# ankitkumar93/compute-war

Hardware: AMD Instinct MI355X
Metric: GB/s ingested (Skein-512 + LZ4, 64 KiB blocks) (higher is better)
Workload: dtype u64; 1 GPU; skein512+lz4, 1048576 x 65536 B uniform-random blocks/GPU in HBM; blocks_per_gpu=1048576, block_bytes=65536, parallelism=block-sharded x1, gather-only RCCL

## Files before the change

### compute_war_amd/csrc/cdc_kernels.hip

```cpp

#include <hip/hip_runtime.h>
#include <stdint.h>

#include "cdc_resolve.h"
#include "cw_device.h"
#include "stream_scratch.h"

namespace cw {

namespace {

constexpr unsigned kScanThreads = 512;

template <bool HI, bool EDGE>
__device__ __forceinline__ void scan_slice(const uint64_t *__restrict__ tab, unsigned copy, const uint8_t *__restrict__ base,
                                           uint64_t last_granule, uint64_t q0, uint64_t off, uint64_t nv, uint64_t ms, uint64_t ml,
                                           uint64_t &ws, uint64_t &wl)
{
    const uint32_t msh = (uint32_t)(ms >> 32), msl = (uint32_t)ms, mlh = (uint32_t)(ml >> 32), mll = (uint32_t)ml;
    auto granule = [&](int i) __attribute__((always_inline)) {
        const int64_t gi = (int64_t)(q0 >> 4) - 4 + i;
        const uint64_t g = gi < 0 ? 0 : ((uint64_t)gi > last_granule ? last_granule : (uint64_t)gi);
        return *reinterpret_cast<const uint4 *>(base + g * 16);
    };
    uint64_t h = 0, s = 0, l = 0;
    uint4 cur = granule(0);
#pragma unroll 1
    for (int i = 0; i < 8; i++) {
        const uint4 nxt = granule(i + 1 < 8 ? i + 1 : 7);
        const uint32_t d[4] = {cur.x, cur.y, cur.z, cur.w};
#pragma unroll
        for (int j = 0; j < 16; j++) {
            const uint32_t b = (d[j >> 2] >> (8 * (j & 3))) & 0xFF;
            uint64_t g = tab[(b << 5) | copy];
            const int pos = 16 * i + j - 64;
// ... 3 lines not shown
                const uint32_t hh = (uint32_t)(h >> 32), hl = (uint32_t)h;
                bool cs = (hh & msh) == 0, cl = (hh & mlh) == 0;
                if (!HI) { cs = cs && (hl & msl) == 0; cl = cl && (hl & mll) == 0; }
                if (EDGE) {
                    const uint64_t q = q0 + pos;
                    const bool in = q >= off && q < nv;
                    cs = cs && in; cl = cl && in;
                }
                s |= (uint64_t)cs << pos;
                l |= (uint64_t)cl << pos;
            }
        }
        cur = nxt;
    }
    ws = s;
    wl = l;
}

template <bool HI>
__global__ void __launch_bounds__(kScanThreads)
cdc_scan_kernel(const uint8_t *__restrict__ base, uint64_t off, uint64_t n, const uint64_t *__restrict__ gear, uint64_t ms, uint64_t ml,
                uint64_t *__restrict__ l0s, uint64_t *__restrict__ l0l, uint64_t *__restrict__ l1, uint64_t nwords, uint64_t nspans)
{
    __shared__ uint64_t tab[256 * 32];
    for (unsigned i = threadIdx.x; i < 256 * 32; i += blockDim.x) tab[i] = gear[i >> 5];
    __syncthreads();
    const unsigned lane = threadIdx.x & 63, copy = threadIdx.x & 31;
    const uint64_t nv = n + off, last_granule = (nv - 1) >> 4;
    const uint64_t waves = (uint64_t)gridDim.x * (kScanThreads / 64);
    for (uint64_t span = (uint64_t)blockIdx.x * (kScanThreads / 64) + (threadIdx.x >> 6); span < nspans; span += waves) {
        const uint64_t word = span * 64 + lane, q0 = word * 64;
        const bool edge = span == 0 || (span + 1) * 4096 > nv;
        uint64_t ws, wl;
        if (edge) scan_slice<HI, true>(tab, copy, base, last_granule, q0, off, nv, ms, ml, ws, wl);
        else scan_slice<HI, false>(tab, copy, base, last_granule, q0, off, nv, ms, ml, ws, wl);
        const bool have = word < nwords;
        if (have) { l0s[word] = ws; l0l[word] = wl; }
        const uint64_t b0 = __ballot(have && ws != 0), b1 = __ballot(have && wl != 0);
        const uint64_t b2 = __ballot(have && ws != ~0ull), b3 = __ballot(have && wl != ~0ull);
        if (lane == 0) {
            l1[span * 4 + 0] = b0; l1[span * 4 + 1] = b1; l1[span * 4 + 2] = b2; l1[span * 4 + 3] = b3;
        }
    }
}

__global__ void __launch_bounds__(256)
cdc_summary_kernel(const uint64_t *__restrict__ in, uint64_t nin, uint64_t *__restrict__ out, uint64_t nout)
// ... 110 lines not shown
    const size_t nstreams = st ? st->nstreams : 0;
    hipError_t e = space.reserve(st ? cdc_streams_workspace_bytes(nbytes, nstreams, p.min_size, seg) : cdc_workspace_bytes(nbytes, p.min_size, seg), kFloor);
    if (e != hipSuccess) return e;
    uint8_t *w = space.as<uint8_t>();
    auto take = [&](size_t bytes) { uint8_t *r = w; w += up256(bytes); return r; };
    uint64_t *gear = reinterpret_cast<uint64_t *>(take(2048));
    uint64_t *l0 = reinterpret_cast<uint64_t *>(take(2 * nwords * 8));
    uint64_t *lv = reinterpret_cast<uint64_t *>(take(4 * 8 * (n1 + n2 + n3)));
    const uint64_t cuts = nseg * cap + nstreams;
    uint64_t *segs = reinterpret_cast<uint64_t *>(take(2 * cuts * 8 + 2 * nseg * 8 + (nseg + 63) / 64 * 8 + 3 * nseg * 4));
    uint64_t *notmerged = segs + 2 * cuts + 2 * nseg;
    uint32_t *counts = reinterpret_cast<uint32_t *>(take(nseg * 4));
    uint64_t *segoff = reinterpret_cast<uint64_t *>(take((nseg + 1) * 8));
    uint32_t *eidx = st ? reinterpret_cast<uint32_t *>(take((nseg + 1) * 4)) : nullptr;

    e = hipMemcpyAsync(gear, p.gear, 2048, hipMemcpyHostToDevice, stream);
    if (e == hipSuccess) e = hipMemsetAsync(notmerged, 0, (nseg + 63) / 64 * 8, stream);
    if (e != hipSuccess) return e;
    if (st) {
        if ((e = cdc_streams_verdict_launch(*st, nbytes, seg, nseg, eidx, offsets, nchunks, stream)) != hipSuccess) return e;
    }
    const bool hi = (uint32_t)p.mask_s == 0 && (uint32_t)p.mask_l == 0;
    const unsigned scan_grid = (unsigned)(n1 < 4096 ? (n1 + 7) / 8 : 512);
    if (hi) hipLaunchKernelGGL((cdc_scan_kernel<true>), dim3(scan_grid), dim3(kScanThreads), 0, stream, base, off, (uint64_t)nbytes, gear,
                               p.mask_s, p.mask_l, l0, l0 + nwords, lv, nwords, n1);
    else hipLaunchKernelGGL((cdc_scan_kernel<false>), dim3(scan_grid), dim3(kScanThreads), 0, stream, base, off, (uint64_t)nbytes, gear,
                            p.mask_s, p.mask_l, l0, l0 + nwords, lv, nwords, n1);
    uint64_t *l1 = lv, *l2 = lv + 4 * n1, *l3 = lv + 4 * (n1 + n2);
    hipLaunchKernelGGL(cdc_summary_kernel, dim3((unsigned)umin((n2 + 3) / 4, 1024)), dim3(256), 0, stream, l1, n1, l2, n2);
    hipLaunchKernelGGL(cdc_summary_kernel, dim3((unsigned)umin((n3 + 3) / 4, 1024)), dim3(256), 0, stream, l2, n2, l3, n3);

    CdcS c;
    c.l0 = l0; c.lv = lv;
    c.nwords = nwords; c.n1 = n1; c.n2 = n2; c.off = off; c.n = nbytes; c.seg = seg; c.nseg = nseg;
    c.m = p.min_size; c.a = p.normal_size; c.M = p.max_size; c.cap = (uint32_t)cap; c.final_ = final_;
    c.segs = segs;
    const unsigned sg = (unsigned)((nseg + 63) / 64), cg = (unsigned)((nseg + 255) / 256);
    if (st) {
        c.ends = st->ends; c.eidx = eidx; c.verdict = st->result; c.nstreams = nstreams;
        if ((e = cdc_streams_resolve_launch(c, counts, stream)) != hipSuccess) return e;
    } else {
        const Cdc &c1 = c;
        hipLaunchKernelGGL(cdc_spec_kernel<Cdc>, dim3(sg), dim3(64), 0, stream, c1, nseg);
        hipLaunchKernelGGL(cdc_merge_kernel<Cdc>, dim3(sg), dim3(64), 0, stream, c1, nseg);
        hipLaunchKernelGGL(cdc_fixup_kernel<Cdc>, dim3(1), dim3(64), 0, stream, c1, nseg);
        hipLaunchKernelGGL(cdc_count_kernel<Cdc>, dim3(cg), dim3(256), 0, stream, c1, nseg, counts);
    }
    e = hipGetLastError();
    if (e != hipSuccess) return e;
// ... 53 lines not shown
```

### compute_war_amd/csrc/cw_api.hip

```cpp

#include <atomic>
#include <cstdarg>
#include <cstdio>
#include <cstdlib>
#include <cstring>
#include <memory>
#include <mutex>
#include <string>
#include <vector>

#include "cw_host.h"
#include "launch_plan.h"

using namespace cw::host;

namespace {
thread_local char t_err[512] = "";

struct ProfSpan { int kind; hipEvent_t a, b; };
thread_local bool t_prof_on = false;
thread_local std::vector<ProfSpan> t_prof;
}

int cw::host::fail(int code, const char *fmt, ...)
// ... 624 lines not shown
{
    int rc = ensure_init();
    if (rc != CW_OK) return rc;
    HIP_TRY(hipMemcpy(dst, d_src, bytes, hipMemcpyDeviceToHost));
    return CW_OK;
}
int cw_dev_synchronize(void)
{
    int rc = ensure_init();
    if (rc != CW_OK) return rc;
    HIP_TRY(hipDeviceSynchronize());
    return CW_OK;
}

#ifdef CW_CLOCK_STAMP
int cw_debug_clock_read(int which, unsigned long long *out)
{
    int rc = ensure_init();
    if (rc != CW_OK) return rc;
    HIP_TRY(hipDeviceSynchronize());
    HIP_TRY(which == 0 ? cw::skein_clock_read(out) : cw::lz4_clock_read(out));
    return CW_OK;
}
#endif

void cw_profile_enable(int on) { t_prof_on = on != 0; }

int cw_profile_read(double ms_sum[3], unsigned count[3], int reset)
{
    for (int k = 0; k < PROF_KINDS; k++) { ms_sum[k] = 0; count[k] = 0; }
    for (ProfSpan &p : t_prof) {
        float ms = 0;
        HIP_TRY(hipEventSynchronize(p.b));
        HIP_TRY(hipEventElapsedTime(&ms, p.a, p.b));
        ms_sum[p.kind] += ms;
        count[p.kind]++;
    }
    if (reset) {
        for (ProfSpan &p : t_prof) { (void)hipEventDestroy(p.a); (void)hipEventDestroy(p.b); }
        t_prof.clear();
    }
    return CW_OK;
}

int cw_profile_kernels(int kind, char *buf, size_t cap)
{
// ... 492 lines not shown
```

### compute_war_amd/csrc/cw_device.h

```cpp
#pragma once

#include <hip/hip_runtime.h>
#include <stddef.h>
#include <stdint.h>

#include "knobs.h"

#ifndef CW_SKEIN_THREADS
#define CW_SKEIN_THREADS 64
#endif

namespace cw {

#ifdef CW_CLOCK_STAMP
constexpr unsigned kClockSlots = 1024;
struct ClockScope {
    unsigned long long m0 = 0, r0 = 0;
    unsigned long long *rec;
    bool on;
    __device__ ClockScope(unsigned long long *buf, unsigned wg) : rec(buf + 4 * (wg % kClockSlots)), on(threadIdx.x == 0)
    {
        if (on) { m0 = __builtin_amdgcn_s_memtime(); r0 = __builtin_amdgcn_s_memrealtime(); }
    }
    __device__ ~ClockScope()
    {
        if (on) {
            const unsigned long long m1 = __builtin_amdgcn_s_memtime(), r1 = __builtin_amdgcn_s_memrealtime();
            rec[0] = m0; rec[1] = r0; rec[2] = m1; rec[3] = r1;
        }
    }
};
#define CW_CLOCK_SCOPE(buf) ClockScope clock_scope_(buf, blockIdx.x)
#define CW_CLOCK_SCOPE_KEYED(buf, key) ClockScope clock_scope_(buf, ((unsigned)(key) % 8u) * 128u + blockIdx.x % 128u)
hipError_t skein_clock_read(unsigned long long *out);
hipError_t lz4_clock_read(unsigned long long *out);
#else
#define CW_CLOCK_SCOPE(buf) do { } while (0)
#define CW_CLOCK_SCOPE_KEYED(buf, key) do { } while (0)
#endif

struct SkeinIV { uint64_t w[8]; };

void note_kernels(int kind, const char *names);
void skein_compute_iv(int state_words, unsigned hash_bits, SkeinIV *iv, uint64_t tree_info = 0);
hipError_t skein_tree_launch(int state_words, const uint8_t *src, size_t block_bytes, size_t src_stride, size_t nblocks,
                             unsigned hash_bits, unsigned leaf, unsigned node, unsigned max_level, uint8_t *digests, hipStream_t stream);

struct HashPlan;
hipError_t skein_launch(const HashPlan &p, const uint8_t *src, size_t block_bytes, size_t src_stride, size_t nblocks, const SkeinIV &iv,
                        uint8_t *digests, unsigned digest_bytes, hipStream_t stream);
hipError_t sha256_launch(const HashPlan &p, const uint8_t *src, size_t block_bytes, size_t src_stride, size_t nblocks, uint8_t *digests,
                         hipStream_t stream);
struct AfterScan { hipError_t (*fn)(void *ctx); void *ctx; };
hipError_t lz4_launch(const uint8_t *src, size_t block_bytes, size_t src_stride, size_t nblocks, uint8_t *dst,
                      size_t dst_stride, uint32_t *sizes, hipStream_t stream, const AfterScan *after_scan = nullptr);
const uint32_t *lz4_queued_blocks_word(hipStream_t stream);
hipError_t lzf_launch(const uint8_t *src, size_t block_bytes, size_t src_stride, size_t nblocks, uint8_t *dst,
                      size_t dst_stride, uint32_t *sizes, hipStream_t stream);
enum class Lz4Vtab : uint8_t;
hipError_t lz4_vtab_launch(Lz4Vtab kernel, uint32_t grid, uint32_t lds, hipStream_t stream, const uint8_t *src, uint32_t n, size_t src_stride, uint8_t *dst,
                           size_t dst_stride, uint32_t *sizes, const uint32_t *queue, uint32_t *counters, uint32_t min_queued, uint32_t max_queued,
// ... 176 lines not shown
```

### compute_war_amd/csrc/launch_plan.h

```cpp
#pragma once

#include <stddef.h>
#include <stdint.h>
#include <stdlib.h>

#include <string>
#include <vector>

#include "knobs.h"

namespace cw {

constexpr uint32_t kTabBytes = (1u << 13) * 2;
constexpr uint32_t kStageMax = 16384;
constexpr uint32_t kFpBytes = (1u << 13) / 2;
constexpr uint32_t kChunk = 4096;
constexpr uint32_t kLzfTabBytes = (1u << 16) * 2;
constexpr uint32_t kInLdsMax = 16384;
constexpr uint32_t kChainMax = 16384;
constexpr uint32_t kShareSpinCap = 1u << 20;

enum class Lz4ScanSpan : uint8_t { unaligned, aligned };
enum class Lz4Parse : uint8_t { global, staged, fp8, fp16, fp32 };
enum class Lz4Lanes : uint8_t { plain, tagged, fp };
enum class Lz4Ring : uint8_t { k1, k2, k4, k8 };
enum class Lz4Blocks : uint8_t { global, staged };
enum class Lz4Vtab : uint8_t { gen2, gen3, lds_table };
enum class LzfLanes : uint8_t { plain, tagged };
enum class LzfChain : uint8_t { small, big, sthread };
enum class LzfParse : uint8_t { global, staged };

template <class E, class Fn>
struct KernelRow { E id; const char *name; Fn *fn; };
template <class E, class Fn, size_t N>
inline const KernelRow<E, Fn> &kernel_row(const KernelRow<E, Fn> (&table)[N], E id)
{
    for (const auto &r : table)
        if (r.id == id) return r;
    abort();
// ... 134 lines not shown
```

### compute_war_amd/csrc/lz4_kernel.hip

```cpp

#include <hip/hip_runtime.h>
#include <stdint.h>
#include <stdio.h>
#include <stdlib.h>
#include <string.h>

#include <optional>
#include <type_traits>

#include "cw_device.h"
#include "lane_codec.h"
#include "launch_plan.h"
#include "lz_device.h"
#include "stream_scratch.h"

#ifndef HEADW_GLOBAL
#define HEADW_GLOBAL 16
#endif
#ifndef HEADW_STAGED
#define HEADW_STAGED 64
#endif

namespace cw {

// ... 43 lines not shown
    const uint32_t n255 = extra / 255;
    for (uint32_t i = lane; i < n255; i += 64) g[i] = 255;
    if (lane == 0) g[n255] = (uint8_t)(extra - n255 * 255);
    return n255 + 1;
}


__device__ __forceinline__ uint32_t ld32g(const uint8_t *p)
{
    uint32_t v;
    __builtin_memcpy(&v, p, 4);
    return v;
}

}

struct ScanState {
    bool hit = false, maybe = false;
    uint32_t mcand = 0, mv = 0;
};

__device__ __forceinline__ uint32_t scan_issue(uint32_t *tab, uint32_t tag, uint32_t pos, uint32_t v, bool active)
{
    const uint32_t h = v * 2654435761u, fp = (h >> 7) & 0xFFFu;
    return atomicMax(&tab[active ? h >> 19 : 0u], active ? tag | (pos << 12) | fp : 0u);
}
__device__ __forceinline__ void scan_judge(uint32_t old, uint32_t epoch, uint32_t v0, uint32_t pos, uint32_t v, bool active, ScanState &st)
{
    const uint32_t fp = ((v * 2654435761u) >> 7) & 0xFFFu, cand = (old >> 12) & 0xFFFFu;
    const bool same = (old >> 28) == epoch;
    const bool fpm = active && same && (old & 0xFFFu) == fp;
    st.hit |= active && (same ? cand >= pos : v == v0);
    st.hit |= fpm && st.maybe;
    st.mcand = fpm ? cand : st.mcand;
    st.mv = fpm ? v : st.mv;
    st.maybe |= fpm;
}

__device__ __forceinline__ bool scan_settle(const uint8_t *g, ScanState &st)
{
    if (__ballot(st.maybe)) {
        if (st.maybe) st.hit |= ld32g(g + st.mcand) == st.mv;
        st.maybe = false;
    }
    return __ballot(st.hit) != 0;
}

__device__ __forceinline__ void scan_begin_block(uint32_t *tab, uint32_t &epoch, uint32_t lane)
{
    if (++epoch == 16) {
        for (uint32_t i = lane; i < (1u << 13) / 4; i += 64) reinterpret_cast<uint4 *>(tab)[i] = make_uint4(0, 0, 0, 0);
        epoch = 1;
    }
}

struct BlockFeed {
// ... 6 lines not shown
        __syncthreads();
        if (lane == 0) *mailbox = atomicAdd(&counters[2], run);
        __syncthreads();
        f.next = __builtin_amdgcn_readfirstlane(*mailbox);
        f.end = f.next + run;
    }
    blk = f.next++;
    return blk < nblocks;
}

__device__ __forceinline__ void scan_mark(uint32_t *sizes, size_t blk, uint32_t *queue, uint32_t *counters, uint32_t lane)
{
    if (lane == 0) {
        sizes[blk] = kNeedsParse;
        queue[atomicAdd(&counters[1], 1u)] = (uint32_t)blk;
    }
}

__global__ void __launch_bounds__(64)
lz4_scan_kernel(const uint8_t *__restrict__ src, uint32_t n, size_t src_stride, size_t nblocks,
                        uint8_t *__restrict__ dst, size_t dst_stride, uint32_t *__restrict__ sizes, uint32_t nprobes,
                        uint32_t *__restrict__ queue, uint32_t *__restrict__ counters)
{
    __shared__ __attribute__((aligned(16))) uint32_t tab[1u << 13];
    __shared__ __attribute__((aligned(16))) uint32_t mailbox_word[4];
    volatile uint32_t *mailbox = mailbox_word;
    const uint32_t lane = threadIdx.x;
    __builtin_amdgcn_s_setprio(3);
    uint32_t epoch = 15;

    BlockFeed feed;
    const uint32_t run = n >= 65536 ? 1u : 65536u / n;
    for (size_t blk; scan_next_block(feed, blk, counters, mailbox, run, nblocks, lane);) {
        scan_begin_block(tab, epoch, lane);
        const uint8_t *g = src + blk * src_stride;
        uint8_t *out = dst + blk * dst_stride;
        const uint32_t tag = epoch << 28;
        ScanState st;
        bool marked = false;

        if (nprobes) {
            const uint32_t v0 = ld32g(g);
            {
                const uint32_t h0 = v0 * 2654435761u;
                if (lane == 0) atomicMax(&tab[h0 >> 19], tag | ((h0 >> 7) & 0xFFFu));
            }
            for (uint32_t k0 = 0; k0 < nprobes && !marked; k0 += 64 * kScanGroup) {
                uint32_t pos[kScanGroup], v[kScanGroup];
                bool act[kScanGroup];
#pragma unroll
                for (int j = 0; j < kScanGroup; j++) {
                    const uint32_t k = k0 + 64 * j + lane;
                    pos[j] = 1 + probe_delta(k);
                    act[j] = k < nprobes;
                    v[j] = ld32g(g + (act[j] ? pos[j] : 0u));
                }
                uint32_t old[kScanGroup];
#pragma unroll
                for (int j = 0; j < kScanGroup; j++) old[j] = scan_issue(tab, tag, pos[j], v[j], act[j]);
#pragma unroll
                for (int j = 0; j < kScanGroup; j++) scan_judge(old[j], epoch, v0, pos[j], v[j], act[j], st);
                marked = scan_settle(g, st);
            }
        }
        if (marked) {
            scan_mark(sizes, blk, queue, counters, lane);
            continue;
        }
        uint32_t op = 1;
        if (n >= 15) {
            if (lane == 0) out[0] = 15u << 4;
            op += put_len(out + 1, n - 15, lane);
        } else if (lane == 0) {
            out[0] = (uint8_t)(n << 4);
        }
        copy_g2g(out + op, g, n, lane);
        if (lane == 0) sizes[blk] = op + n;
    }
}

constexpr uint32_t kPieces = kChunk / 1024, kRing = 2 * kChunk, kStreamGroup = 2;

struct Chunk { uint4 p[kPieces]; };

__device__ __forceinline__ void chunk_load(Chunk &r, const uint8_t *g, uint32_t c, uint32_t nchunks, uint32_t n, uint32_t lane)
{
#pragma unroll
    for (uint32_t j = 0; j < kPieces; j++) {
        const uint32_t off = c * kChunk + j * 1024 + lane * 16;
        if (c < nchunks && off < n) r.p[j] = *reinterpret_cast<const uint4 *>(g + off);
    }
}
__device__ __forceinline__ void chunk_stage(const Chunk &r, uint32_t *ring32, uint32_t c, uint32_t n, uint32_t lane)
{
#pragma unroll
    for (uint32_t j = 0; j < kPieces; j++) {
        const uint32_t off = c * kChunk + j * 1024 + lane * 16;
        if (off < n) *reinterpret_cast<uint4 *>(reinterpret_cast<uint8_t *>(ring32) + (off & (kRing - 1))) = r.p[j];
    }
}
__device__ __forceinline__ void chunk_store(const Chunk &r, uint8_t *lit, uint32_t c, uint32_t n, uint32_t lane)
{
#pragma unroll
    for (uint32_t j = 0; j < kPieces; j++) {
// ... 40 lines not shown
        for (uint32_t j = 0; j < kStreamGroup; j++) {
            const uint32_t k = w.knext + 64 * j + lane;
            pos[j] = 1 + probe_delta(k);
            act[j] = k < nprobes && pos[j] < end;
            const unsigned long long m = __ballot(act[j]);
            nact += (uint32_t)__builtin_popcountll(m);
            ngroups += m != 0;
        }
        if (nact == 0) return;
        if (ngroups == 1) probe_groups<1>(w, pos, act, tab, ring32, tag, epoch);
        else if (ngroups == 2) probe_groups<2>(w, pos, act, tab, ring32, tag, epoch);
        else probe_groups<kStreamGroup>(w, pos, act, tab, ring32, tag, epoch);
        w.marked = scan_settle(g, w.st);
        w.knext += nact;
        if (w.marked || nact < 64 * kStreamGroup) return;
    }
}

__global__ void __launch_bounds__(64)
lz4_scan_stream_kernel(const uint8_t *__restrict__ src, uint32_t n, size_t src_stride, size_t nblocks,
                       uint8_t *__restrict__ dst, size_t dst_stride, uint32_t *__restrict__ sizes, uint32_t nprobes,
                       uint32_t *__restrict__ queue, uint32_t *__restrict__ counters, size_t first_block, uint32_t feed_word)
{
    __shared__ __attribute__((aligned(16))) uint32_t tab[1u << 13];
    __shared__ __attribute__((aligned(16))) uint32_t ring32[kRing / 4];
    volatile uint32_t *mailbox = ring32;
    const uint32_t lane = threadIdx.x;
    __builtin_amdgcn_s_setprio(3);
    uint32_t epoch = 15;
    const uint32_t nchunks = (n + kChunk - 1) / kChunk;
    const uint32_t hdr = 1 + (n >= 15 ? (n - 15) / 255 + 1 : 0);

    BlockFeed feed;
    const uint32_t run = n >= 65536 ? 1u : 65536u / n;
    for (size_t rel; scan_next_block(feed, rel, counters + feed_word - 2, mailbox, run, nblocks - first_block, lane);) {
        const size_t blk = first_block + rel;
        scan_begin_block(tab, epoch, lane);
        const uint8_t *g = src + blk * src_stride;
        uint8_t *out = dst + blk * dst_stride, *lit = out + hdr;
        const uint32_t tag = epoch << 28;
        Walk w;
        Chunk r0, r1, r2;

#define CW_STAGE(PREV, CUR, C)                                                                         \
        do {                                                                                           \
            const uint32_t c_ = (C);                                                                   \
            if (c_) chunk_store(PREV, lit, c_ - 1, n, lane);                                           \
            chunk_load(PREV, g, c_ + 2, nchunks, n, lane);                                             \
            chunk_stage(CUR, ring32, c_, n, lane);                                                     \
            if (c_ == 0) {                                                                             \
                w.v0 = ring32[0];                                                                      \
                if (nprobes && lane == 0) {                                                            \
                    const uint32_t h0 = w.v0 * 2654435761u;                                            \
                    atomicMax(&tab[h0 >> 19], tag | ((h0 >> 7) & 0xFFFu));             \
                }                                                                                      \
            } else {                                                                                   \
                probe_upto(w, c_ * kChunk, tab, ring32, tag, epoch, nprobes, g, lane);                 \
            }                                                                                          \
// ... 114 lines not shown
    w.marked = probe_batches<1, true>(pos, q ? 0u : 62u, left < 64 ? left : 64u, tab, ring32, tag, w.v0, g, lane);
    w.qnext = q + 1;
}

__device__ __forceinline__ void probe_range(SpanWalk &w, uint32_t qe, uint32_t *tab, const uint32_t *ring32, uint32_t tag, const uint8_t *g,
                                            uint32_t lane)
{
    uint32_t q = w.qnext;
    w.qnext = qe;
    uint32_t p = __umul24(q, lane) + group_base(q);
    for (; q + 2 <= qe; q += 2) {
        const uint32_t pos[2] = {p, p + lane + (64 * q + 1)};
        if (probe_batches<2, false>(pos, 0, 64, tab, ring32, tag, w.v0, g, lane)) { w.marked = true; return; }
        p = pos[1] + lane + (64 * q + 65);
    }
    if (q < qe) {
        const uint32_t pos[1] = {p};
        w.marked = probe_batches<1, false>(pos, 0, 64, tab, ring32, tag, w.v0, g, lane);
    }
}

#ifdef CW_CLOCK_STAMP
__device__ unsigned long long g_clock_scan[4 * kClockSlots];
hipError_t lz4_clock_read(unsigned long long *out) { return hipMemcpyFromSymbol(out, HIP_SYMBOL(g_clock_scan), sizeof g_clock_scan); }
#endif

template <bool ALIGNED>
__global__ void __launch_bounds__(64)
lz4_scan_span_kernel(const uint8_t *__restrict__ src, uint32_t n, size_t src_stride, uint32_t nspans, uint8_t *__restrict__ dst,
                     size_t dst_stride, uint32_t *__restrict__ sizes, uint32_t nprobes, uint32_t *__restrict__ queue,
                     uint32_t *__restrict__ counters, uint32_t lg)
{
    CW_CLOCK_SCOPE(g_clock_scan);
    __shared__ __attribute__((aligned(16))) uint32_t tab[1u << 13];
    __shared__ __attribute__((aligned(16))) uint32_t ring32[kRing / 4];
    volatile uint32_t *mailbox = ring32;
    const uint32_t lane = threadIdx.x;
    __builtin_amdgcn_s_setprio(3);
    uint32_t epoch = 15;
    const uint32_t cmask = (1u << lg) - 1, run = 16u >> lg;
    const uint32_t hdr = 1 + (n - 15) / 255 + 1;
    const uint32_t lane16 = lane * 16;
    const uint32_t qlast = (nprobes + 61) >> 6;
    const uint32_t gend = group_end((lane + 1) * kChunk < n ? (lane + 1) * kChunk : n, qlast);
    const uint32_t hdrw = (0xFFu << 16) | (((n - 15) % 255) << 24);

    for (;;) {
        __syncthreads();
        if (lane == 0) *mailbox = atomicAdd(&counters[2], 1u);
        __syncthreads();
        const uint32_t span = __builtin_amdgcn_readfirstlane(*mailbox);
        if (span >= nspans) break;
        __syncthreads();
        const size_t first = (size_t)span * run;
        const uint8_t *gs = src + first * src_stride;
        uint8_t *os = dst + first * dst_stride + (ALIGNED ? hdr - 2 : hdr);

        SpanWalk w;
// ... 851 lines not shown
        blk = queue[qi];
        g = src + (size_t)blk * src_stride;
        out = dst + (size_t)blk * dst_stride;
        return Take::kTaken;
    }
};

template <int MODE>
__global__ void __launch_bounds__(64)
lz4_lanes_kernel(const uint8_t *__restrict__ src, uint32_t n, size_t src_stride, uint8_t *__restrict__ dst, size_t dst_stride,
                 uint32_t *__restrict__ sizes, const uint32_t *__restrict__ queue, uint32_t *__restrict__ counters,
                 uint16_t *__restrict__ tables, uint32_t min_blocks, uint32_t reserve)
{
    const uint32_t qcount = counters[1];
    if (qcount < min_blocks) return;
    if ((size_t)blockIdx.x * 64 >= qcount) return;
    LaneQueue s{src, src_stride, dst, dst_stride, sizes, queue, counters, qcount, reserve, n, n - kMFLimit, n - kLastLiterals,
                src, dst, 0};
    LaneTab<MODE> t{reinterpret_cast<typename LaneTab<MODE>::Entry *>(tables) + ((size_t)blockIdx.x * 64 + threadIdx.x) * (1u << 13)};
    lz4_lane_run(s, t);
}

constexpr uint32_t kRingBytes = 256, kRingPiece = 64;
enum : uint32_t { LB_NEXT = 0, LB_PROBE = 1, LB_EXTEND = 2, LB_TAIL = 3, LB_EXIT = 4 };

template <int K>
__device__ __forceinline__ void
lz4_lanes_ring_body(uint32_t *__restrict__ ring, const uint32_t qcount, const uint8_t *__restrict__ src, uint32_t n, size_t src_stride, uint8_t *__restrict__ dst,
                    size_t dst_stride, uint32_t *__restrict__ sizes, const uint32_t *__restrict__ queue, uint32_t *__restrict__ counters,
                    uint16_t *__restrict__ tables, uint32_t reserve)
{
    const uint32_t lane = threadIdx.x;
    uint32_t *tab = reinterpret_cast<uint32_t *>(tables) + ((size_t)blockIdx.x * 64 + lane) * (1u << 13);
    const uint32_t mflimit = n - kMFLimit, matchlimit = n - kLastLiterals;

    auto ring_dw = [&](uint32_t x) -> uint32_t { return ring[((x >> 2) & (kRingBytes / 4 - 1)) * 64 + lane]; };
    auto ring32 = [&](uint32_t x) -> uint32_t { return __builtin_amdgcn_alignbyte(ring_dw(x + 4), ring_dw(x), x & 3u); };
    auto ring16 = [&](uint32_t x) -> uint4 {
        const uint32_t d0 = ring_dw(x), d1 = ring_dw(x + 4), d2 = ring_dw(x + 8), d3 = ring_dw(x + 12), d4 = ring_dw(x + 16), r = x & 3u;
        return make_uint4(__builtin_amdgcn_alignbyte(d1, d0, r), __builtin_amdgcn_alignbyte(d2, d1, r), __builtin_amdgcn_alignbyte(d3, d2, r),
                          __builtin_amdgcn_alignbyte(d4, d3, r));
    };

    uint32_t state = LB_NEXT;
    const uint8_t *g = src;
    uint8_t *out = dst;
// ... 228 lines not shown
            const uint32_t run = n - anchor;
            if (run >= 15) { out[op++] = 15u << 4; lane_put_len(out, op, run - 15); }
            else out[op++] = (uint8_t)(run << 4);
            uint32_t k = 0;
            for (; k + 16 <= run; k += 16) {
                uint4 q;
                __builtin_memcpy(&q, g + anchor + k, 16);
                __builtin_memcpy(out + op + k, &q, 16);
            }
            for (; k < run; k++) out[op + k] = g[anchor + k];
            op += run;
            sizes[blk] = op;
            state = LB_NEXT;
        }
    }
}

template <int K>
__global__ void __launch_bounds__(64)
lz4_lanes_ring_kernel(const uint8_t *__restrict__ src, uint32_t n, size_t src_stride, uint8_t *__restrict__ dst, size_t dst_stride,
                      uint32_t *__restrict__ sizes, const uint32_t *__restrict__ queue, uint32_t *__restrict__ counters,
                      uint16_t *__restrict__ tables, uint32_t min_blocks, uint32_t reserve, uint32_t max_blocks)
{
    __shared__ uint32_t ring[(kRingBytes / 4) * 64];
    const uint32_t qcount = counters[1];
    if (qcount < min_blocks || qcount >= max_blocks) return;
    if ((size_t)blockIdx.x * 64 >= qcount) return;
    lz4_lanes_ring_body<K>(ring, qcount, src, n, src_stride, dst, dst_stride, sizes, queue, counters, tables, reserve);
}

__global__ void __launch_bounds__(64)
lz4_lanes_ring_auto_kernel(const uint8_t *__restrict__ src, uint32_t n, size_t src_stride, uint8_t *__restrict__ dst, size_t dst_stride,
                           uint32_t *__restrict__ sizes, const uint32_t *__restrict__ queue, uint32_t *__restrict__ counters,
                           uint16_t *__restrict__ tables, uint32_t min_blocks, uint32_t reserve_mid, uint32_t wide_from, uint32_t reserve_wide,
                           uint32_t leave_mid)
{
    __shared__ uint32_t ring[(kRingBytes / 4) * 64];
    const uint32_t qcount = counters[1];
    if (qcount < min_blocks) return;
    if ((size_t)blockIdx.x * 64 >= qcount) return;
    if (qcount >= wide_from) {
        lz4_lanes_ring_body<1>(ring, qcount, src, n, src_stride, dst, dst_stride, sizes, queue, counters, tables, reserve_wide);
    } else {
        if ((size_t)blockIdx.x * 64 + leave_mid >= qcount && blockIdx.x > 0) return;
        lz4_lanes_ring_body<2>(ring, qcount, src, n, src_stride, dst, dst_stride, sizes, queue, counters, tables, reserve_mid);
    }
}

namespace {
struct Workspace {
    DeviceBuf queues;
    DeviceBuf lane_tabs;
    SideStream lanes;
    SideStream vtab;
    void release() { (void)queues.release(); (void)lane_tabs.release(); lanes.release(); vtab.release(); }
};
StreamScratch<Workspace> workspaces;
}

const uint32_t *lz4_queued_blocks_word(hipStream_t stream)
// ... 50 lines not shown
    if (!lz4_call_valid(block_bytes, nblocks)) return hipErrorInvalidValue;
    const uint32_t n = (uint32_t)block_bytes;
    const Knobs kn = knobs();
    const CodecCall call = codec_call(src, block_bytes, src_stride, nblocks, dst, dst_stride);
    Lz4Plan p = lz4_plan(call, kn);
    hipError_t e = lz4_set_attributes();
    if (e != hipSuccess) return e;
    auto &wsp = workspaces.at(stream);
    LaunchLock sequence(wsp.launch);
    if ((e = wsp.queues.reserve(p.queue_bytes, p.queue_min_bytes)) != hipSuccess) return e;
    if (p.lanes.on && wsp.lane_tabs.reserve(p.lane_tab_bytes) != hipSuccess) {
        (void)hipGetLastError();
        p = lz4_plan(call, kn, false);
    }
    const size_t cap = (wsp.queues.bytes() / sizeof(uint32_t) - 8) / 2;
    uint32_t *counters = wsp.queues.as<uint32_t>(), *queue = counters + 8, *queue2 = queue + cap;
    uint16_t *const lane_tabs = wsp.lane_tabs.as<uint16_t>();
    std::optional<SideStream::Fork> lanes_fork, vtab_fork;
    auto on = [&](const Stage &s) { return s.stream == Target::lanes_side ? wsp.lanes.stream : s.stream == Target::vtab_side ? wsp.vtab.stream : stream; };
    auto pool = [](SidePool sp) { return sp == SidePool::greatest ? SideStream::greatest : SideStream::normal; };

    if ((e = hipMemsetAsync(counters, 0, 8 * sizeof(uint32_t), stream)) != hipSuccess) return e;
    if (p.scan_span.on)
        hipLaunchKernelGGL(kernel_row(kScanSpanKernels, p.scan_span_kernel).fn, dim3(p.scan_span.grid), dim3(64), 0, stream, src, n, src_stride, p.nspans,
                           dst, dst_stride, sizes, scan_probes(n), queue, counters, p.lg);
    if (p.scan_stream.on)
        hipLaunchKernelGGL(lz4_scan_stream_kernel, dim3(p.scan_stream.grid), dim3(64), 0, stream, src, n, src_stride, nblocks, dst,
                           dst_stride, sizes, scan_probes(n), queue, counters, p.done, 3u);
    if (p.scan_generic.on)
        hipLaunchKernelGGL(lz4_scan_kernel, dim3(p.scan_generic.grid), dim3(64), 0, stream, src, n, src_stride, nblocks, dst,
                           dst_stride, sizes, scan_probes(n), queue, counters);
    if ((e = hipGetLastError()) != hipSuccess) return e;
    if (after_scan && (e = after_scan->fn(after_scan->ctx)) != hipSuccess) return e;
    if (p.stop_after_scan) { note_kernels(0, describe(p).text); return hipSuccess; }
    if (p.lanes.on) {
        if (p.lanes.stream == Target::lanes_side) {
            if ((e = wsp.lanes.open(pool(p.lanes_pool))) != hipSuccess) return e;
            if ((e = lanes_fork.emplace(wsp.lanes, stream).err) != hipSuccess) return e;
        }
        const dim3 lgrid(p.lanes.grid);
        if (p.lanes_form == Lz4Plan::LanesForm::ring_auto)
            hipLaunchKernelGGL(lz4_lanes_ring_auto_kernel, lgrid, dim3(64), 0, on(p.lanes), src, n, src_stride, dst, dst_stride, sizes, queue, counters,
                               lane_tabs, p.lmin, p.reserve, p.wide_from, p.reserve_wide, p.lane_leave);
        else if (p.lanes_form == Lz4Plan::LanesForm::ring)
            hipLaunchKernelGGL(kernel_row(kRingKernels, p.ring_kernel).fn, lgrid, dim3(64), 0, on(p.lanes), src, n, src_stride, dst, dst_stride, sizes, queue,
                               counters, lane_tabs, p.lmin, p.reserve, kNoMax);
        else
            hipLaunchKernelGGL(kernel_row(kLanesKernels, p.lanes_kernel).fn, lgrid, dim3(64), 0, on(p.lanes), src, n, src_stride, dst, dst_stride, sizes, queue,
                               counters, lane_tabs, p.lmin, p.reserve);
        if ((e = hipGetLastError()) != hipSuccess) return e;
    }
    if (p.vtab.on) {
        if (p.vtab.stream == Target::vtab_side) {
            if ((e = wsp.vtab.open(pool(p.vtab_pool))) != hipSuccess) return e;
            if ((e = vtab_fork.emplace(wsp.vtab, stream).err) != hipSuccess) return e;
        }
        if ((e = lz4_vtab_launch(p.vtab_kernel, p.vtab.grid, p.vtab.lds, on(p.vtab), src, n, src_stride, dst, dst_stride, sizes, queue, counters, p.vmin, p.vmax,
                                 p.vres)) != hipSuccess) return e;
    }
    if (p.ltab.on && (e = lz4_vtab_launch(Lz4Vtab::lds_table, p.ltab.grid, p.ltab.lds, stream, src, n, src_stride, dst, dst_stride, sizes, queue, counters, 0u,
                                          kNoMax, 0u)) != hipSuccess) return e;
    if (p.parse.on) {
        hipLaunchKernelGGL(kernel_row(kParseKernels, p.parse_kernel).fn, dim3(p.parse.grid), dim3(64), p.parse.lds, stream, src, n, src_stride, nblocks, dst,
                           dst_stride, sizes, queue, counters, queue2, p.force_redo);
        if ((e = hipGetLastError()) != hipSuccess) return e;
    }
    if (vtab_fork && (e = vtab_fork->join()) != hipSuccess) return e;
    if (lanes_fork && (e = lanes_fork->join()) != hipSuccess) return e;
// ... 9 lines not shown
```

### compute_war_amd/csrc/skein_kernels.hip

```cpp

#include <hip/hip_runtime.h>
#include <stdint.h>
#include <stdlib.h>
#include <string.h>

#include "cw_device.h"
#include "launch_plan.h"
#include "stream_scratch.h"

namespace cw {

#define KS_PARITY 0x5555555555555555ULL

template <int R>
static __device__ __forceinline__ uint64_t rotl(uint64_t x)
{
    const uint32_t lo = (uint32_t)x, hi = (uint32_t)(x >> 32);
    uint32_t nlo, nhi;
    if (R == 32) { nlo = hi; nhi = lo; }
    else if (R < 32) {
        nlo = __builtin_amdgcn_alignbit(lo, hi, 32 - R);
        nhi = __builtin_amdgcn_alignbit(hi, lo, 32 - R);
    } else {
        nlo = __builtin_amdgcn_alignbit(hi, lo, 64 - R);
// ... 269 lines not shown
        fetch_half(S, first + SPL + HS);
        run_half(B, first + HS);
#pragma unroll
        for (unsigned j = 0; j < HS; j++)
#pragma unroll
            for (int k = 0; k < NW; k++) B[j][k] = S[j][k];
    }

    uint8_t *out = digests + gid * digest_bytes;
    if (((digest_bytes | (unsigned)reinterpret_cast<uintptr_t>(out)) & 15) == 0) {
        uint4 *o4 = reinterpret_cast<uint4 *>(out);
#pragma unroll
        for (int k = 0; k < NW / 2; k++)
            if ((unsigned)(16 * k) < digest_bytes)
                o4[k] = make_uint4((uint32_t)X[2 * k], (uint32_t)(X[2 * k] >> 32), (uint32_t)X[2 * k + 1], (uint32_t)(X[2 * k + 1] >> 32));
    } else {
        for (unsigned k = 0; k < digest_bytes; k++) out[k] = (uint8_t)(X[k >> 3] >> (8 * (k & 7)));
    }
}


#ifdef CW_CLOCK_STAMP
__device__ unsigned long long g_clock_skein[4 * kClockSlots];
hipError_t skein_clock_read(unsigned long long *out) { return hipMemcpyFromSymbol(out, HIP_SYMBOL(g_clock_skein), sizeof g_clock_skein); }
#endif

template <int NW, bool ALIGNED16, bool INTERIOR>
__global__ void __launch_bounds__(CW_SKEIN_THREADS)
skein_slice_kernel(const uint8_t *__restrict__ src, size_t block_bytes, size_t src_stride, size_t nblocks, SkeinIV iv,
                   uint8_t *__restrict__ digests, unsigned digest_bytes, uint64_t *__restrict__ state, size_t s_begin, size_t s_end)
{
    CW_CLOCK_SCOPE_KEYED(g_clock_skein, s_begin / (s_end - s_begin ? s_end - s_begin : 1));
    constexpr unsigned BB = NW * 8, SPL = 128 / BB, HS = SPL / 2;
    const size_t gid = (size_t)blockIdx.x * blockDim.x + threadIdx.x;
    if (gid >= nblocks) return;
    const uint8_t *p = src + gid * src_stride;
    const size_t nmsg = block_bytes / BB, total = nmsg + 1;
    uint64_t *st = state + gid * NW;

    uint64_t X[NW];
    if (s_begin == 0) {
#pragma unroll
        for (int i = 0; i < NW; i++) X[i] = iv.w[i];
    } else {
#pragma unroll
        for (int i = 0; i < NW; i++) X[i] = st[i];
    }
    uint64_t t0 = (uint64_t)s_begin * BB, t1 = (s_begin == 0 ? T1_FIRST : 0) | T1_MSG;

    uint64_t A[HS][NW], B[HS][NW], S[HS][NW];
    auto fetch_half = [&](uint64_t (&dst)[HS][NW], size_t first) __attribute__((always_inline)) {
#pragma unroll
        for (unsigned j = 0; j < HS; j++) {
            const size_t s = first + j;
            if constexpr (INTERIOR) {
// ... 353 lines not shown
```

Baseline: 1156 GB/s.

## Move kernel LDS to dynamic shared memory and add clock census instrumentation

Converts the static shared arrays in the CDC scan, LZ4 scan and ring-lane kernels to dynamically sized extern shared memory, with the sizes passed at launch, and registers LDS limits for the CDC scan kernel. Rewrites the scan hash-table issue and judge helpers with branchless masks and bitwise booleans, and uses empty asm barriers to keep the lane id in a vector register. Adds a debug census recorder, enabled only under the clock-stamp build flag, that captures per-workgroup hardware IDs and timestamps. The likely intent is to cut scalar/vector branching overhead and control how shared memory is allocated, at the cost of extra complexity and a risk of mismatched LDS sizes.

```diff
diff --git a/compute_war_amd/csrc/cdc_kernels.hip b/compute_war_amd/csrc/cdc_kernels.hip
--- a/compute_war_amd/csrc/cdc_kernels.hip
+++ b/compute_war_amd/csrc/cdc_kernels.hip
@@ -11,6 +11,7 @@
 namespace {
 
 constexpr unsigned kScanThreads = 512;
+constexpr uint32_t kScanLds = 256 * 32 * 8;
 
 template <bool HI, bool EDGE>
 __device__ __forceinline__ void scan_slice(const uint64_t *__restrict__ tab, unsigned copy, const uint8_t *__restrict__ base,
@@ -60,7 +61,8 @@
 cdc_scan_kernel(const uint8_t *__restrict__ base, uint64_t off, uint64_t n, const uint64_t *__restrict__ gear, uint64_t ms, uint64_t ml,
                 uint64_t *__restrict__ l0s, uint64_t *__restrict__ l0l, uint64_t *__restrict__ l1, uint64_t nwords, uint64_t nspans)
 {
-    __shared__ uint64_t tab[256 * 32];
+    extern __shared__ __attribute__((aligned(16))) uint8_t smem[];
+    uint64_t *const tab = reinterpret_cast<uint64_t *>(smem);
     for (unsigned i = threadIdx.x; i < 256 * 32; i += blockDim.x) tab[i] = gear[i >> 5];
     __syncthreads();
     const unsigned lane = threadIdx.x & 63, copy = threadIdx.x & 31;
@@ -217,9 +219,12 @@
     }
     const bool hi = (uint32_t)p.mask_s == 0 && (uint32_t)p.mask_l == 0;
     const unsigned scan_grid = (unsigned)(n1 < 4096 ? (n1 + 7) / 8 : 512);
-    if (hi) hipLaunchKernelGGL((cdc_scan_kernel<true>), dim3(scan_grid), dim3(kScanThreads), 0, stream, base, off, (uint64_t)nbytes, gear,
+    static std::atomic<bool> lds_set{false};
+    if ((e = set_lds_limits_once(lds_set, {{reinterpret_cast<const void *>(cdc_scan_kernel<true>), kScanLds},
+                                           {reinterpret_cast<const void *>(cdc_scan_kernel<false>), kScanLds}})) != hipSuccess) return e;
+    if (hi) hipLaunchKernelGGL((cdc_scan_kernel<true>), dim3(scan_grid), dim3(kScanThreads), kScanLds, stream, base, off, (uint64_t)nbytes, gear,
                                p.mask_s, p.mask_l, l0, l0 + nwords, lv, nwords, n1);
-    else hipLaunchKernelGGL((cdc_scan_kernel<false>), dim3(scan_grid), dim3(kScanThreads), 0, stream, base, off, (uint64_t)nbytes, gear,
+    else hipLaunchKernelGGL((cdc_scan_kernel<false>), dim3(scan_grid), dim3(kScanThreads), kScanLds, stream, base, off, (uint64_t)nbytes, gear,
                             p.mask_s, p.mask_l, l0, l0 + nwords, lv, nwords, n1);
     uint64_t *l1 = lv, *l2 = lv + 4 * n1, *l3 = lv + 4 * (n1 + n2);
     hipLaunchKernelGGL(cdc_summary_kernel, dim3((unsigned)umin((n2 + 3) / 4, 1024)), dim3(256), 0, stream, l1, n1, l2, n2);
diff --git a/compute_war_amd/csrc/cw_api.hip b/compute_war_amd/csrc/cw_api.hip
--- a/compute_war_amd/csrc/cw_api.hip
+++ b/compute_war_amd/csrc/cw_api.hip
@@ -670,6 +670,14 @@
     HIP_TRY(which == 0 ? cw::skein_clock_read(out) : cw::lz4_clock_read(out));
     return CW_OK;
 }
+int cw_debug_census_read(int which, unsigned long long *out)
+{
+    int rc = ensure_init();
+    if (rc != CW_OK) return rc;
+    HIP_TRY(hipDeviceSynchronize());
+    HIP_TRY(which == 0 ? cw::skein_census_read(out) : cw::lz4_census_read(out));
+    return CW_OK;
+}
 #endif
 
 void cw_profile_enable(int on) { t_prof_on = on != 0; }
diff --git a/compute_war_amd/csrc/cw_device.h b/compute_war_amd/csrc/cw_device.h
--- a/compute_war_amd/csrc/cw_device.h
+++ b/compute_war_amd/csrc/cw_device.h
@@ -14,29 +14,39 @@
 
 #ifdef CW_CLOCK_STAMP
 constexpr unsigned kClockSlots = 1024;
+constexpr unsigned kCensusScan = 1024, kCensusHashLaunch = 16384, kCensusHash = 8 * kCensusHashLaunch;
 struct ClockScope {
-    unsigned long long m0 = 0, r0 = 0;
-    unsigned long long *rec;
+    unsigned long long m0 = 0, r0 = 0, where = 0;
+    unsigned long long *rec, *cen;
     bool on;
-    __device__ ClockScope(unsigned long long *buf, unsigned wg) : rec(buf + 4 * (wg % kClockSlots)), on(threadIdx.x == 0)
+    __device__ ClockScope(unsigned long long *buf, unsigned wg, unsigned long long *census)
+        : rec(buf + 4 * (wg % kClockSlots)), cen(census), on(threadIdx.x == 0)
     {
-        if (on) { m0 = __builtin_amdgcn_s_memtime(); r0 = __builtin_amdgcn_s_memrealtime(); }
+        if (on) {
+            where = (unsigned long long)__builtin_amdgcn_s_getreg((31 << 11) | 4) | (unsigned long long)__builtin_amdgcn_s_getreg((31 << 11) | 20) << 32;
+            m0 = __builtin_amdgcn_s_memtime(); r0 = __builtin_amdgcn_s_memrealtime();
+        }
     }
     __device__ ~ClockScope()
     {
         if (on) {
             const unsigned long long m1 = __builtin_amdgcn_s_memtime(), r1 = __builtin_amdgcn_s_memrealtime();
             rec[0] = m0; rec[1] = r0; rec[2] = m1; rec[3] = r1;
+            cen[0] = r0; cen[1] = r1; cen[2] = m1 - m0; cen[3] = where;
         }
     }
 };
-#define CW_CLOCK_SCOPE(buf) ClockScope clock_scope_(buf, blockIdx.x)
-#define CW_CLOCK_SCOPE_KEYED(buf, key) ClockScope clock_scope_(buf, ((unsigned)(key) % 8u) * 128u + blockIdx.x % 128u)
+#define CW_CLOCK_SCOPE(buf, census) ClockScope clock_scope_(buf, blockIdx.x, (census) + 4 * (blockIdx.x % kCensusScan))
+#define CW_CLOCK_SCOPE_KEYED(buf, census, key)                                                \
+    ClockScope clock_scope_(buf, ((unsigned)(key) % 8u) * 128u + blockIdx.x % 128u,           \
+                            (census) + 4 * (((unsigned)(key) % 8u) * kCensusHashLaunch + blockIdx.x % kCensusHashLaunch))
 hipError_t skein_clock_read(unsigned long long *out);
 hipError_t lz4_clock_read(unsigned long long *out);
+hipError_t skein_census_read(unsigned long long *out);
+hipError_t lz4_census_read(unsigned long long *out);
 #else
-#define CW_CLOCK_SCOPE(buf) do { } while (0)
-#define CW_CLOCK_SCOPE_KEYED(buf, key) do { } while (0)
+#define CW_CLOCK_SCOPE(buf, census) do { } while (0)
+#define CW_CLOCK_SCOPE_KEYED(buf, census, key) do { } while (0)
 #endif
 
 struct SkeinIV { uint64_t w[8]; };
diff --git a/compute_war_amd/csrc/launch_plan.h b/compute_war_amd/csrc/launch_plan.h
--- a/compute_war_amd/csrc/launch_plan.h
+++ b/compute_war_amd/csrc/launch_plan.h
@@ -15,6 +15,10 @@
 constexpr uint32_t kStageMax = 16384;
 constexpr uint32_t kFpBytes = (1u << 13) / 2;
 constexpr uint32_t kChunk = 4096;
+constexpr uint32_t kRing = 2 * kChunk;
+constexpr uint32_t kScanTabBytes = (1u << 13) * 4;
+constexpr uint32_t kScanSpanLds = kScanTabBytes + kRing, kScanStreamLds = kScanTabBytes + kRing, kScanGenericLds = kScanTabBytes + 16;
+constexpr uint32_t kLaneRingLds = 256 * 64;
 constexpr uint32_t kLzfTabBytes = (1u << 16) * 2;
 constexpr uint32_t kInLdsMax = 16384;
 constexpr uint32_t kChainMax = 16384;
diff --git a/compute_war_amd/csrc/lz4_kernel.hip b/compute_war_amd/csrc/lz4_kernel.hip
--- a/compute_war_amd/csrc/lz4_kernel.hip
+++ b/compute_war_amd/csrc/lz4_kernel.hip
@@ -89,16 +89,16 @@
 
 __device__ __forceinline__ uint32_t scan_issue(uint32_t *tab, uint32_t tag, uint32_t pos, uint32_t v, bool active)
 {
-    const uint32_t h = v * 2654435761u, fp = (h >> 7) & 0xFFFu;
-    return atomicMax(&tab[active ? h >> 19 : 0u], active ? tag | (pos << 12) | fp : 0u);
+    const uint32_t h = v * 2654435761u, fp = (h >> 7) & 0xFFFu, on = active ? ~0u : 0u;
+    return atomicMax(&tab[(h >> 19) & on], (tag | (pos << 12) | fp) & on);
 }
 __device__ __forceinline__ void scan_judge(uint32_t old, uint32_t epoch, uint32_t v0, uint32_t pos, uint32_t v, bool active, ScanState &st)
 {
     const uint32_t fp = ((v * 2654435761u) >> 7) & 0xFFFu, cand = (old >> 12) & 0xFFFFu;
     const bool same = (old >> 28) == epoch;
-    const bool fpm = active && same && (old & 0xFFFu) == fp;
-    st.hit |= active && (same ? cand >= pos : v == v0);
-    st.hit |= fpm && st.maybe;
+    const bool fpm = active & same & ((old & 0xFFFu) == fp);
+    st.hit |= active & ((same & (cand >= pos)) | (!same & (v == v0)));
+    st.hit |= fpm & st.maybe;
     st.mcand = fpm ? cand : st.mcand;
     st.mv = fpm ? v : st.mv;
     st.maybe |= fpm;
@@ -151,9 +151,9 @@
                         uint8_t *__restrict__ dst, size_t dst_stride, uint32_t *__restrict__ sizes, uint32_t nprobes,
                         uint32_t *__restrict__ queue, uint32_t *__restrict__ counters)
 {
-    __shared__ __attribute__((aligned(16))) uint32_t tab[1u << 13];
-    __shared__ __attribute__((aligned(16))) uint32_t mailbox_word[4];
-    volatile uint32_t *mailbox = mailbox_word;
+    extern __shared__ __attribute__((aligned(16))) uint8_t smem[];
+    uint32_t *const tab = reinterpret_cast<uint32_t *>(smem);
+    volatile uint32_t *mailbox = reinterpret_cast<uint32_t *>(smem + kScanTabBytes);
     const uint32_t lane = threadIdx.x;
     __builtin_amdgcn_s_setprio(3);
     uint32_t epoch = 15;
@@ -163,7 +163,6 @@
     for (size_t blk; scan_next_block(feed, blk, counters, mailbox, run, nblocks, lane);) {
         scan_begin_block(tab, epoch, lane);
         const uint8_t *g = src + blk * src_stride;
-        uint8_t *out = dst + blk * dst_stride;
         const uint32_t tag = epoch << 28;
         ScanState st;
         bool marked = false;
@@ -196,19 +195,21 @@
             scan_mark(sizes, blk, queue, counters, lane);
             continue;
         }
-        uint32_t op = 1;
+        uint8_t *out = dst + blk * dst_stride;
+        uint32_t op = 1, ln = lane;
+        asm volatile("" : "+v"(ln));
         if (n >= 15) {
-            if (lane == 0) out[0] = 15u << 4;
-            op += put_len(out + 1, n - 15, lane);
-        } else if (lane == 0) {
+            if (ln == 0) out[0] = 15u << 4;
+            op += put_len(out + 1, n - 15, ln);
+        } else if (ln == 0) {
             out[0] = (uint8_t)(n << 4);
         }
-        copy_g2g(out + op, g, n, lane);
-        if (lane == 0) sizes[blk] = op + n;
-    }
-}
-
-constexpr uint32_t kPieces = kChunk / 1024, kRing = 2 * kChunk, kStreamGroup = 2;
+        copy_g2g(out + op, g, n, ln);
+        if (ln == 0) sizes[blk] = op + n;
+    }
+}
+
+constexpr uint32_t kPieces = kChunk / 1024, kStreamGroup = 2;
 
 struct Chunk { uint4 p[kPieces]; };
 
@@ -295,10 +296,10 @@
                        uint8_t *__restrict__ dst, size_t dst_stride, uint32_t *__restrict__ sizes, uint32_t nprobes,
                        uint32_t *__restrict__ queue, uint32_t *__restrict__ counters, size_t first_block, uint32_t feed_word)
 {
-    __shared__ __attribute__((aligned(16))) uint32_t tab[1u << 13];
-    __shared__ __attribute__((aligned(16))) uint32_t ring32[kRing / 4];
+    extern __shared__ __attribute__((aligned(16))) uint8_t smem[];
+    uint32_t *const tab = reinterpret_cast<uint32_t *>(smem), *const ring32 = reinterpret_cast<uint32_t *>(smem + kScanTabBytes);
     volatile uint32_t *mailbox = ring32;
-    const uint32_t lane = threadIdx.x;
+    const uint32_t lane0 = threadIdx.x;
     __builtin_amdgcn_s_setprio(3);
     uint32_t epoch = 15;
     const uint32_t nchunks = (n + kChunk - 1) / kChunk;
@@ -306,7 +307,9 @@
 
     BlockFeed feed;
     const uint32_t run = n >= 65536 ? 1u : 65536u / n;
-    for (size_t rel; scan_next_block(feed, rel, counters + feed_word - 2, mailbox, run, nblocks - first_block, lane);) {
+    for (size_t rel; scan_next_block(feed, rel, counters + feed_word - 2, mailbox, run, nblocks - first_block, lane0);) {
+        uint32_t lane = lane0;
+        asm volatile("" : "+v"(lane));
         const size_t blk = first_block + rel;
         scan_begin_block(tab, epoch, lane);
         const uint8_t *g = src + blk * src_stride;
@@ -467,7 +470,9 @@
 
 #ifdef CW_CLOCK_STAMP
 __device__ unsigned long long g_clock_scan[4 * kClockSlots];
+__device__ unsigned long long g_census_scan[4 * kCensusScan];
 hipError_t lz4_clock_read(unsigned long long *out) { return hipMemcpyFromSymbol(out, HIP_SYMBOL(g_clock_scan), sizeof g_clock_scan); }
+hipError_t lz4_census_read(unsigned long long *out) { return hipMemcpyFromSymbol(out, HIP_SYMBOL(g_census_scan), sizeof g_census_scan); }
 #endif
 
 template <bool ALIGNED>
@@ -476,9 +481,9 @@
                      size_t dst_stride, uint32_t *__restrict__ sizes, uint32_t nprobes, uint32_t *__restrict__ queue,
                      uint32_t *__restrict__ counters, uint32_t lg)
 {
-    CW_CLOCK_SCOPE(g_clock_scan);
-    __shared__ __attribute__((aligned(16))) uint32_t tab[1u << 13];
-    __shared__ __attribute__((aligned(16))) uint32_t ring32[kRing / 4];
+    CW_CLOCK_SCOPE(g_clock_scan, g_census_scan);
+    extern __shared__ __attribute__((aligned(16))) uint8_t smem[];
+    uint32_t *const tab = reinterpret_cast<uint32_t *>(smem), *const ring32 = reinterpret_cast<uint32_t *>(smem + kScanTabBytes);
     volatile uint32_t *mailbox = ring32;
     const uint32_t lane = threadIdx.x;
     __builtin_amdgcn_s_setprio(3);
@@ -1376,6 +1381,7 @@
 }
 
 constexpr uint32_t kRingBytes = 256, kRingPiece = 64;
+static_assert(kLaneRingLds == kRingBytes * 64, "the ring lanes' LDS: kRingBytes per lane");
 enum : uint32_t { LB_NEXT = 0, LB_PROBE = 1, LB_EXTEND = 2, LB_TAIL = 3, LB_EXIT = 4 };
 
 template <int K>
@@ -1650,7 +1656,8 @@
                       uint32_t *__restrict__ sizes, const uint32_t *__restrict__ queue, uint32_t *__restrict__ counters,
                       uint16_t *__restrict__ tables, uint32_t min_blocks, uint32_t reserve, uint32_t max_blocks)
 {
-    __shared__ uint32_t ring[(kRingBytes / 4) * 64];
+    extern __shared__ __attribute__((aligned(16))) uint8_t smem[];
+    uint32_t *const ring = reinterpret_cast<uint32_t *>(smem);
     const uint32_t qcount = counters[1];
     if (qcount < min_blocks || qcount >= max_blocks) return;
     if ((size_t)blockIdx.x * 64 >= qcount) return;
@@ -1663,7 +1670,8 @@
                            uint16_t *__restrict__ tables, uint32_t min_blocks, uint32_t reserve_mid, uint32_t wide_from, uint32_t reserve_wide,
                            uint32_t leave_mid)
 {
-    __shared__ uint32_t ring[(kRingBytes / 4) * 64];
+    extern __shared__ __attribute__((aligned(16))) uint8_t smem[];
+    uint32_t *const ring = reinterpret_cast<uint32_t *>(smem);
     const uint32_t qcount = counters[1];
     if (qcount < min_blocks) return;
     if ((size_t)blockIdx.x * 64 >= qcount) return;
@@ -1760,13 +1768,13 @@
 
     if ((e = hipMemsetAsync(counters, 0, 8 * sizeof(uint32_t), stream)) != hipSuccess) return e;
     if (p.scan_span.on)
-        hipLaunchKernelGGL(kernel_row(kScanSpanKernels, p.scan_span_kernel).fn, dim3(p.scan_span.grid), dim3(64), 0, stream, src, n, src_stride, p.nspans,
+        hipLaunchKernelGGL(kernel_row(kScanSpanKernels, p.scan_span_kernel).fn, dim3(p.scan_span.grid), dim3(64), kScanSpanLds, stream, src, n, src_stride, p.nspans,
                            dst, dst_stride, sizes, scan_probes(n), queue, counters, p.lg);
     if (p.scan_stream.on)
-        hipLaunchKernelGGL(lz4_scan_stream_kernel, dim3(p.scan_stream.grid), dim3(64), 0, stream, src, n, src_stride, nblocks, dst,
+        hipLaunchKernelGGL(lz4_scan_stream_kernel, dim3(p.scan_stream.grid), dim3(64), kScanStreamLds, stream, src, n, src_stride, nblocks, dst,
                            dst_stride, sizes, scan_probes(n), queue, counters, p.done, 3u);
     if (p.scan_generic.on)
-        hipLaunchKernelGGL(lz4_scan_kernel, dim3(p.scan_generic.grid), dim3(64), 0, stream, src, n, src_stride, nblocks, dst,
+        hipLaunchKernelGGL(lz4_scan_kernel, dim3(p.scan_generic.grid), dim3(64), kScanGenericLds, stream, src, n, src_stride, nblocks, dst,
                            dst_stride, sizes, scan_probes(n), queue, counters);
     if ((e = hipGetLastError()) != hipSuccess) return e;
     if (after_scan && (e = after_scan->fn(after_scan->ctx)) != hipSuccess) return e;
@@ -1778,10 +1786,10 @@
         }
         const dim3 lgrid(p.lanes.grid);
         if (p.lanes_form == Lz4Plan::LanesForm::ring_auto)
-            hipLaunchKernelGGL(lz4_lanes_ring_auto_kernel, lgrid, dim3(64), 0, on(p.lanes), src, n, src_stride, dst, dst_stride, sizes, queue, counters,
+            hipLaunchKernelGGL(lz4_lanes_ring_auto_kernel, lgrid, dim3(64), kLaneRingLds, on(p.lanes), src, n, src_stride, dst, dst_stride, sizes, queue, counters,
                                lane_tabs, p.lmin, p.reserve, p.wide_from, p.reserve_wide, p.lane_leave);
         else if (p.lanes_form == Lz4Plan::LanesForm::ring)
-            hipLaunchKernelGGL(kernel_row(kRingKernels, p.ring_kernel).fn, lgrid, dim3(64), 0, on(p.lanes), src, n, src_stride, dst, dst_stride, sizes, queue,
+            hipLaunchKernelGGL(kernel_row(kRingKernels, p.ring_kernel).fn, lgrid, dim3(64), kLaneRingLds, on(p.lanes), src, n, src_stride, dst, dst_stride, sizes, queue,
                                counters, lane_tabs, p.lmin, p.reserve, kNoMax);
         else
             hipLaunchKernelGGL(kernel_row(kLanesKernels, p.lanes_kernel).fn, lgrid, dim3(64), 0, on(p.lanes), src, n, src_stride, dst, dst_stride, sizes, queue,
diff --git a/compute_war_amd/csrc/skein_kernels.hip b/compute_war_amd/csrc/skein_kernels.hip
--- a/compute_war_amd/csrc/skein_kernels.hip
+++ b/compute_war_amd/csrc/skein_kernels.hip
@@ -315,7 +315,9 @@
 
 #ifdef CW_CLOCK_STAMP
 __device__ unsigned long long g_clock_skein[4 * kClockSlots];
+__device__ unsigned long long g_census_skein[4 * kCensusHash];
 hipError_t skein_clock_read(unsigned long long *out) { return hipMemcpyFromSymbol(out, HIP_SYMBOL(g_clock_skein), sizeof g_clock_skein); }
+hipError_t skein_census_read(unsigned long long *out) { return hipMemcpyFromSymbol(out, HIP_SYMBOL(g_census_skein), sizeof g_census_skein); }
 #endif
 
 template <int NW, bool ALIGNED16, bool INTERIOR>
@@ -323,7 +325,7 @@
 skein_slice_kernel(const uint8_t *__restrict__ src, size_t block_bytes, size_t src_stride, size_t nblocks, SkeinIV iv,
                    uint8_t *__restrict__ digests, unsigned digest_bytes, uint64_t *__restrict__ state, size_t s_begin, size_t s_end)
 {
-    CW_CLOCK_SCOPE_KEYED(g_clock_skein, s_begin / (s_end - s_begin ? s_end - s_begin : 1));
+    CW_CLOCK_SCOPE_KEYED(g_clock_skein, g_census_skein, s_begin / (s_end - s_begin ? s_end - s_begin : 1));
     constexpr unsigned BB = NW * 8, SPL = 128 / BB, HS = SPL / 2;
     const size_t gid = (size_t)blockIdx.x * blockDim.x + threadIdx.x;
     if (gid >= nblocks) return;
```

Result: no change. 1155 GB/s (-0.0%).
